# leok7v/sqz

Measured on AMD Instinct MI355X. Metric: encode MB/s + decode MB/s, 32KB window, batched blocks, 1/2/4/8 MI355X, higher is better.
Workload: dtype u8; 1 GPU; 4096 x 262144 B Zipf(s=1) byte blocks, window 2^15, one independent stream per block (BASELINE.json configs[2]); total_blocks=4096, blocks_per_gpu=4096, block_bytes=262144, win_bits=15, parallelism=1 rank; the N>1 runs shard this same batch (strong scaling), finder=index, device=AMD Radeon Graphics (gfx950:sramecc+:xnack-)

## Files before the change

sqz_amd/csrc/lz77_index.hip:

```cpp
#include "sqz_device.h"
#include "sqz_kernels.h"

namespace sqzk {

constexpr int kSharedGiveUp = 8;
constexpr int kXcds = 8;
constexpr int kSortThreads = 1024;
constexpr int kSortWaves = kSortThreads / kWave;

constexpr int kSortTile = 4 * kSortThreads;

constexpr int kSortBins = 1024;
constexpr int kSortCntRow = kSortBins + 2;
struct SortLds {
    uint32_t elem[kSortTile];
    uint16_t dig[kSortTile];
    uint16_t cnt[kSortWaves][kSortCntRow];
    uint32_t gbase[3][kSortBins];
    uint32_t delta[kSortBins];
    uint32_t wtot[kSortWaves];
};

struct __attribute__((packed)) U32u { uint32_t v; };

__device__ __forceinline__ uint32_t load_u32_unaligned(const uint8_t* p) {
    return reinterpret_cast<const U32u*>(p)->v;
}

__device__ __forceinline__ uint64_t peers_of(uint32_t digit, bool valid, int bits) {
    const uint64_t all = __ballot(valid);
    uint32_t lo = (uint32_t)all, hi = (uint32_t)(all >> 32);
#pragma unroll
    for (int bit = 0; bit < 10; bit++) {
        if (bit < bits) {
            const uint32_t mine = (uint32_t)((int32_t)(digit << (31 - bit)) >> 31);
            const uint64_t m = __ballot(mine != 0u);
            lo &= ~((uint32_t)m ^ mine);
            hi &= ~((uint32_t)(m >> 32) ^ mine);
        }
    }
    return ((uint64_t)hi << 32) | lo;
}

__device__ __forceinline__ uint32_t lanes_below(uint64_t mask) {
    return __builtin_amdgcn_mbcnt_hi((uint32_t)(mask >> 32),
                                     __builtin_amdgcn_mbcnt_lo((uint32_t)mask, 0u));
}

__device__ __forceinline__ uint32_t sort_key(const uint8_t* src, uint64_t bytes, uint32_t k) {
    return (uint64_t)k + 4 <= bytes ? (__builtin_bswap32(load_u32_unaligned(src + k)) >> 8)
                                    : (((uint32_t)src[k] << 16) | ((uint32_t)src[k + 1] << 8) | (uint32_t)src[k + 2]);
}

typedef uint32_t __attribute__((may_alias)) SortCntPair;

struct SortSec {
#ifdef SQZ_STATS
    uint64_t t[8] = {0, 0, 0, 0, 0, 0, 0, 0};
    uint64_t last = 0;
#endif
};
#ifdef SQZ_STATS
#define SORT_SEC(s, k) { const uint64_t n_ = __builtin_readcyclecounter(); (s).t[k] += n_ - (s).last; (s).last = n_; }
#define SORT_SEC_LOADS(s, k) { asm volatile("s_waitcnt vmcnt(0)" ::: "memory"); SORT_SEC(s, k) }
#else
#define SORT_SEC(s, k)
#define SORT_SEC_LOADS(s, k)
#endif

template <int kBits, bool kSmall>
__device__ __forceinline__ void sort_pass(SortLds& lds, const int pass, const uint8_t* __restrict__ src,
                                          const uint64_t bytes, const uint32_t count, const bool carry,
                                          const uint32_t* __restrict__ from, uint32_t* __restrict__ to, SortSec& sec) {
    constexpr int kDigits = 1 << kBits;
    constexpr int kTpd = kSortThreads / kDigits;
    constexpr int kWpt = kSortWaves / kTpd;
    const int tid = threadIdx.x;
    const int lane = tid & (kWave - 1);
    const int wave = __builtin_amdgcn_readfirstlane(tid >> 6);
    const bool first = kSmall ? kBits == 10 : pass == 0;
    uint32_t* const gbase = lds.gbase[pass];

    auto fetch = [&](uint32_t tile, uint32_t (&raw)[4]) {
#pragma unroll
        for (int j = 0; j < 4; j++) {
            const uint32_t k = tile + (uint32_t)(wave * 256 + j * kWave + lane);
            if (first) {
                const uint32_t last = (uint32_t)(bytes - 4);
                raw[j] = load_u32_unaligned(src + (k < last ? k : last));
            } else {
                raw[j] = from[k < count ? k : count - 1u];
            }
        }
    };
    auto key_from = [&](uint32_t raw, uint32_t k) {
        const uint32_t be = __builtin_bswap32(raw);
        return (uint64_t)k + 4 <= bytes ? be >> 8 : be & 0x00FFFFFFu;
    };
    auto decode = [&](uint32_t tile, const uint32_t (&raw)[4], uint32_t (&elem)[4], uint32_t (&digit)[4], bool (&valid)[4]) {
#pragma unroll
        for (int j = 0; j < 4; j++) {
            const uint32_t k = tile + (uint32_t)(wave * 256 + j * kWave + lane);
            valid[j] = k < count;
            const uint32_t pos = valid[j] ? (first ? k : raw[j]) : 0u;
            digit[j] = 0; elem[j] = pos;
            if (!valid[j]) { continue; }
            if (kSmall) {
                if (first) {
                    const uint32_t key = key_from(raw[j], k);
                    digit[j] = key & 0x3FFu;
                    elem[j] = pos | ((key >> 10) << 18);
                } else if (pass == 1) {
                    digit[j] = (pos >> 18) & 0x7Fu;
                } else {
                    digit[j] = pos >> 25;
                    elem[j] = pos & 0x3FFFFu;
                }
            } else if (first) {
                digit[j] = key_from(raw[j], k) & 0xFFu;
            } else if (pass == 1) {
                const uint32_t w = (uint32_t)src[pos] | ((uint32_t)src[pos + 1] << 8);
                digit[j] = w >> 8;
                if (carry) { elem[j] = pos | ((w & 0xFFu) << 24); }
            } else {
                digit[j] = carry ? (pos >> 24) : (uint32_t)src[pos];
                if (carry) { elem[j] = pos & 0x00FFFFFFu; }
            }
        }
    };

    uint32_t ahead[4], elem[4], digit[4], wrank[4];
    bool valid[4];
    fetch(0u, ahead);
    decode(0u, ahead, elem, digit, valid);
    SORT_SEC_LOADS(sec, 1)
    for (uint32_t tile = 0; tile < count; tile += (uint32_t)kSortTile) {
        const uint32_t n_tile = count - tile < (uint32_t)kSortTile ? count - tile : (uint32_t)kSortTile;
        fetch(tile + (uint32_t)kSortTile, ahead);
        {
            SortCntPair* const row = reinterpret_cast<SortCntPair*>(lds.cnt[wave]);
            for (int d = lane; d < kDigits / 2; d += kWave) { row[d] = 0u; }
        }
#pragma unroll
        for (int j = 0; j < 4; j++) {
            const uint64_t peers = peers_of(digit[j], valid[j], kBits);
            const uint32_t rank = lanes_below(peers);
            wrank[j] = valid[j] ? (uint32_t)lds.cnt[wave][digit[j]] + rank : 0u;
            __builtin_amdgcn_wave_barrier();
            if (valid[j] && rank == 0) {
                lds.cnt[wave][digit[j]] = (uint16_t)(lds.cnt[wave][digit[j]] + (uint32_t)__builtin_popcountll(peers));
            }
            __builtin_amdgcn_wave_barrier();
        }
        lds_barrier();
        SORT_SEC(sec, 2)
        const int sd = tid / kTpd;
        const int sw = (tid % kTpd) * kWpt;
        uint32_t c[kWpt], sum = 0;
#pragma unroll
        for (int i = 0; i < kWpt; i++) { c[i] = lds.cnt[sw + i][sd]; sum += c[i]; }
        const uint32_t incl = wave_scan(sum);
        if (lane == kWave - 1) { lds.wtot[wave] = incl; }
        lds_barrier();
        SORT_SEC(sec, 3)
        uint32_t at = wave_scan(lane < wave ? lds.wtot[lane] : 0u);
        at = (uint32_t)__builtin_amdgcn_readlane((int)at, kWave - 1) + incl - sum;
        const uint32_t run = at;
#pragma unroll
        for (int i = 0; i < kWpt; i++) { lds.cnt[sw + i][sd] = (uint16_t)at; at += c[i]; }
        const uint32_t run_end = kTpd > 1 ? (uint32_t)__shfl((int)at, lane | (kTpd - 1)) : at;
        if (tid % kTpd == 0) {
            const uint32_t g = gbase[sd];
            lds.delta[sd] = g - run;
            gbase[sd] = g + (run_end - run);
        }
        lds_barrier();
        SORT_SEC(sec, 4)
#pragma unroll
        for (int j = 0; j < 4; j++) {
            if (valid[j]) {
                const uint32_t slot = (uint32_t)lds.cnt[wave][digit[j]] + wrank[j];
                if (slot < (uint32_t)kSortTile) {
                    lds.elem[slot] = elem[j];
                    lds.dig[slot] = (uint16_t)digit[j];
                }
            }
        }
        lds_barrier();
        SORT_SEC(sec, 5)
#pragma unroll
        for (int j = 0; j < 4; j++) {
            const uint32_t slot = (uint32_t)(j * kSortThreads + tid);
            const uint32_t s = slot < n_tile ? slot : n_tile - 1u;
            const uint32_t dest = s + lds.delta[lds.dig[s]];
            to[dest < count ? dest : count - 1u] = lds.elem[s];
        }
        SORT_SEC(sec, 6)
        decode(tile + (uint32_t)kSortTile, ahead, elem, digit, valid);
        SORT_SEC_LOADS(sec, 1)
    }
    __threadfence_block();
    __syncthreads();
}

__global__ __launch_bounds__(kSortThreads)
void index_sort_kernel(const uint8_t* __restrict__ in,
                       const uint64_t* __restrict__ in_off,
                       uint32_t n_blocks,
                       uint32_t* __restrict__ buf_a,
                       uint32_t* __restrict__ buf_b,
                       uint64_t slots) {
    __shared__ SortLds lds;
    const uint32_t b = blockIdx.x;
    if (b >= n_blocks || in_off[b + 1] > slots) { return; }
    const int tid = threadIdx.x;
    const int lane = tid & (kWave - 1);
    const int wave = __builtin_amdgcn_readfirstlane(tid >> 6);

    const uint8_t* src = in + in_off[b];
    const uint64_t bytes = in_off[b + 1] - in_off[b];
    if (bytes < 3) { return; }
    const uint32_t count = (uint32_t)(bytes - 2);
    uint32_t* const pa = buf_a + in_off[b];
    uint32_t* const pb = buf_b + in_off[b];
    if (bytes == 3) {
        if (tid == 0) { pa[0] = 0u; }
        return;
    }
    const bool small = bytes <= (1u << 18);
    const bool carry = bytes <= (1u << 24);
    const int w0 = small ? 10 : 8, w1 = small ? 7 : 8, w2 = small ? 7 : 8;
    const int s1 = w0, s2 = w0 + w1;
    const uint32_t m0 = (1u << w0) - 1u, m1 = (1u << w1) - 1u;
    SortSec sec;
#ifdef SQZ_STATS
    sec.last = __builtin_readcyclecounter();
    const uint64_t sec_begin = sec.last;
#endif
    for (int d = tid; d < 3 * kSortBins; d += kSortThreads) { (&lds.gbase[0][0])[d] = 0; }
    __syncthreads();
    auto count_key = [&](uint32_t key) {
        atomicAdd(&lds.gbase[0][key & m0], 1u);
        atomicAdd(&lds.gbase[1][(key >> s1) & m1], 1u);
        atomicAdd(&lds.gbase[2][key >> s2], 1u);
    };
    const uint32_t quads = bytes >= 8 ? (uint32_t)((bytes - 8) / 4) + 1u : 0u;
    if ((uint32_t)tid < quads) {
        uint32_t lo = load_u32_unaligned(src + 4u * (uint32_t)tid), hi = load_u32_unaligned(src + 4u * (uint32_t)tid + 4u);
        for (uint32_t q = (uint32_t)tid; q < quads; q += (uint32_t)kSortThreads) {
            const uint64_t eight = ((uint64_t)hi << 32) | lo;
            const uint32_t nq = q + (uint32_t)kSortThreads < quads ? q + (uint32_t)kSortThreads : q;
            lo = load_u32_unaligned(src + 4u * nq); hi = load_u32_unaligned(src + 4u * nq + 4u);
#pragma unroll
            for (int j = 0; j < 4; j++) { count_key(__builtin_bswap32((uint32_t)(eight >> (8 * j))) >> 8); }
        }
    }
    for (uint32_t k = 4u * quads + (uint32_t)tid; k < count; k += (uint32_t)kSortThreads) { count_key(sort_key(src, bytes, k)); }
    __syncthreads();
    if (wave < 3) {
        uint32_t* const g = lds.gbase[wave];
        const int per = (1 << (wave == 0 ? w0 : wave == 1 ? w1 : w2)) / kWave;
        uint32_t sum = 0;
        for (int j = 0; j < per; j++) { sum += g[per * lane + j]; }
        uint32_t excl = wave_scan(sum) - sum;
        for (int j = 0; j < per; j++) { const uint32_t v = g[per * lane + j]; g[per * lane + j] = excl; excl += v; }
    }
    __syncthreads();
    SORT_SEC(sec, 0)

    if (small) {
        sort_pass<10, true>(lds, 0, src, bytes, count, carry, pb, pa, sec);
        for (int pass = 1; pass < 3; pass++) {
            sort_pass<7, true>(lds, pass, src, bytes, count, carry, pass == 1 ? pa : pb, pass == 1 ? pb : pa, sec);
        }
    } else {
        for (int pass = 0; pass < 3; pass++) {
            sort_pass<8, false>(lds, pass, src, bytes, count, carry, pass == 1 ? pa : pb, pass == 1 ? pb : pa, sec);
        }
    }
#ifdef SQZ_STATS
    if (tid == 0 && b == 1) {
        printf("sort block 1: cycles %llu: hist %llu; tiles: loads %llu rank %llu scan_a %llu scan_b %llu place %llu copy_out %llu\n",
               (unsigned long long)(sec.last - sec_begin), (unsigned long long)sec.t[0], (unsigned long long)sec.t[1],
               (unsigned long long)sec.t[2], (unsigned long long)sec.t[3], (unsigned long long)sec.t[4],
               (unsigned long long)sec.t[5], (unsigned long long)sec.t[6]);
    }
#endif
}

__global__ __launch_bounds__(256)
void index_match_kernel(const uint8_t* __restrict__ in,
                        const uint64_t* __restrict__ in_off,
                        uint32_t n_blocks, uint32_t window,
                        const uint32_t* __restrict__ sorted,
                        uint32_t* __restrict__ match, uint32_t groups, uint64_t slots) {
    const uint32_t xcd = blockIdx.x % (uint32_t)kXcds;
    const uint32_t local = blockIdx.x / (uint32_t)kXcds;
    const uint32_t b = (local / groups) * (uint32_t)kXcds + xcd;
    const uint32_t group = local % groups;
    if (b >= n_blocks || in_off[b + 1] > slots) { return; }
    const uint8_t* src = in + in_off[b];
    const uint64_t bytes = in_off[b + 1] - in_off[b];
    if (bytes < 3) { return; }
    const uint32_t n = (uint32_t)bytes;
    const uint32_t count = n - 2;
    const uint32_t* S = sorted + in_off[b];
    uint32_t* M = match + in_off[b];

    const int lane = (int)(threadIdx.x & (kWave - 1));
    const uint32_t pages = (count + (uint32_t)kWave - 1u) / (uint32_t)kWave;
    const uint32_t waves = groups * (blockDim.x / (uint32_t)kWave);
    const uint32_t per_wave = (pages + waves - 1u) / waves;
    const uint32_t wave_id = group * (blockDim.x / (uint32_t)kWave) + (threadIdx.x - (uint32_t)lane) / (uint32_t)kWave;
    const uint32_t page_lo = wave_id * per_wave;
    const uint32_t page_hi = page_lo + per_wave < pages ? page_lo + per_wave : pages;
    auto load16 = [&](uint32_t at, uint32_t& w0, uint32_t& w1, uint32_t& w2, uint32_t& w3) {
        if (at + 16 <= n) {
            w0 = load_u32_unaligned(src + at); w1 = load_u32_unaligned(src + at + 4);
            w2 = load_u32_unaligned(src + at + 8); w3 = load_u32_unaligned(src + at + 12);
        } else {
            uint32_t w[4] = {0, 0, 0, 0};
            for (uint32_t k = 0; k < 16 && at + k < n; k++) { w[k >> 2] |= (uint32_t)src[at + k] << (8 * (k & 3)); }
            w0 = w[0]; w1 = w[1]; w2 = w[2]; w3 = w[3];
        }
    };
    uint32_t prev_i = 0, prev0 = 0, prev1 = 0, prev2 = 0, prev3 = 0;
    if (page_lo > 0 && page_lo < page_hi) {
        prev_i = S[(page_lo - 1u) * (uint32_t)kWave + (uint32_t)lane];
        load16(prev_i, prev0, prev1, prev2, prev3);
    }
    for (uint32_t pg = page_lo; pg < page_hi; pg++) {
        const uint32_t r0 = pg * (uint32_t)kWave;
        const bool have_prev = pg > 0;
        const uint32_t r = r0 + (uint32_t)lane;
        const bool valid = r < count;
        const uint32_t i = valid ? S[r] : 0u;
        const uint32_t cap = (n - i) < (uint32_t)kLenMax ? (n - i) : (uint32_t)kLenMax;
        const uint32_t reach = i < window - 1 ? i : window - 1;
        uint32_t own0 = 0, own1 = 0, own2 = 0, own3 = 0;
        if (valid) { load16(i, own0, own1, own2, own3); }
        const uint32_t key = own0 & 0x00FFFFFFu;
        uint32_t best = 0, dist = 0;
        auto walk = [&](uint32_t q_from) {
            if (q_from == 0 || best >= cap) { return; }
            auto inside = [&](uint32_t r) {
                const uint32_t p = S[r];
                if (p + 4 > n) { return false; }
                return (load_u32_unaligned(src + p) & 0x00FFFFFFu) == key && i - p <= reach;
            };
            uint32_t q_lo;
            {
                uint32_t d = 4, bad = 0, good = q_from;
                bool open = true;
                while (open) {
                    if (d >= q_from) { bad = 0; open = false; if (inside(0)) { good = 0; } else { bad = 1; } }
                    else if (inside(q_from - d)) { good = q_from - d; d <<= 1; }
                    else { bad = q_from - d + 1; open = false; }
                }
                uint32_t lo = bad, hi = good;
                while (lo < hi) {
                    const uint32_t mid = lo + ((hi - lo) >> 1);
                    if (inside(mid)) { hi = mid; } else { lo = mid + 1; }
                }
                q_lo = lo;
            }
            uint8_t own_next = best >= (uint32_t)kLenMin ? src[i + best] : (uint8_t)0;
            for (uint32_t q = q_from; q > q_lo && best < cap; ) {
                q--;
                const uint32_t p = S[q];
                if (best >= (uint32_t)kLenMin && src[p + best] != own_next) { continue; }
                uint32_t k = 3;
                while (k < cap) {
                    if (i + k + 4 <= n) {
                        const uint32_t x = load_u32_unaligned(src + p + k) ^ load_u32_unaligned(src + i + k);
                        if (x != 0) { k += (uint32_t)__builtin_ctz(x) >> 3; break; }
                        k += 4;
                    } else {
                        if (src[p + k] != src[i + k]) { break; }
                        k++;
                    }
                }
                if (k > cap) { k = cap; }
                if (k > best) {
                    best = k; dist = i - p;
                    if (best < cap) { own_next = src[i + best]; }
                }
            }
        };
        const uint32_t key0 = (uint32_t)__builtin_amdgcn_readfirstlane((int)key);
        if (__ballot(valid && key == key0 && i + 16 <= n) == ~0ull) {
            bool done = false, deferred = false;
            uint32_t resume = 0;
            uint32_t page_base = r0, page = i, pb0 = own0, pb1 = own1, pb2 = own2, pb3 = own3;
            for (int64_t c = (int64_t)r0 + kWave - 2; c >= 0; c--) {
                if (c < (int64_t)page_base) {
                    page_base -= (uint32_t)kWave;
                    page = S[page_base + (uint32_t)lane];
                    load16(page, pb0, pb1, pb2, pb3);
                }
                const int at = (int)(c - (int64_t)page_base);
                const uint32_t pc = (uint32_t)__builtin_amdgcn_readlane((int)page, at);
                const bool below = (int64_t)r > c;
                const uint32_t d = i - pc;
                if (below && d > reach) { done = true; }
                if (__ballot(!done) == 0) { break; }
                const uint32_t c0 = (uint32_t)__builtin_amdgcn_readlane((int)pb0, at);
                if ((c0 & 0x00FFFFFFu) != key0) { break; }
                const uint32_t c1 = (uint32_t)__builtin_amdgcn_readlane((int)pb1, at);
                const uint32_t c2 = (uint32_t)__builtin_amdgcn_readlane((int)pb2, at);
                const uint32_t c3 = (uint32_t)__builtin_amdgcn_readlane((int)pb3, at);
                const uint32_t x0 = own0 ^ c0, x1 = own1 ^ c1, x2 = own2 ^ c2, x3 = own3 ^ c3;
                uint32_t len = x0 != 0 ? ((uint32_t)__builtin_ctz(x0) >> 3)
                             : x1 != 0 ? 4u + ((uint32_t)__builtin_ctz(x1) >> 3)
                             : x2 != 0 ? 8u + ((uint32_t)__builtin_ctz(x2) >> 3)
                             : x3 != 0 ? 12u + ((uint32_t)__builtin_ctz(x3) >> 3) : 16u;
                const bool want = below && !done;
                if (want && len == 16u && cap > 16u) {
                    deferred = true;
                    resume = (uint32_t)c + 1u;
                    done = true;
                } else {
                    if (len > cap) { len = cap; }
                    if (want && len > best) {
                        best = len; dist = d;
                        if (best >= cap) { done = true; }
                    }
                }
                if (__builtin_popcountll(__ballot(deferred)) >= kSharedGiveUp) {
                    if (!done) {
                        deferred = true;
                        resume = below ? (uint32_t)c : r;
                        done = true;
                    }
                    break;
                }
            }
            if (deferred) { walk(resume); }
            M[i] = best >= (uint32_t)kLenMin ? ((best << 16) | dist) : (key & 0xFFu);
            prev_i = i; prev0 = own0; prev1 = own1; prev2 = own2; prev3 = own3;
            continue;
        }
        bool done = !valid;
        bool later = false;
        uint32_t resume = 0;
        for (int k = 1; k <= kWave; k++) {
            const int from = lane - k;
            const bool in_cur = from >= 0;
            if (!done && !in_cur && !have_prev) { done = true; }
            if (__ballot(!done) == 0) { break; }
            const int addr = (from & (kWave - 1)) << 2;
            uint32_t pc = (uint32_t)__builtin_amdgcn_ds_bpermute(addr, (int)i);
            uint32_t c0 = (uint32_t)__builtin_amdgcn_ds_bpermute(addr, (int)own0);
            uint32_t c1 = (uint32_t)__builtin_amdgcn_ds_bpermute(addr, (int)own1);
            const bool back = __ballot(!done && !in_cur) != 0;
            if (back) {
                const uint32_t qc = (uint32_t)__builtin_amdgcn_ds_bpermute(addr, (int)prev_i);
                const uint32_t q0 = (uint32_t)__builtin_amdgcn_ds_bpermute(addr, (int)prev0);
                const uint32_t q1 = (uint32_t)__builtin_amdgcn_ds_bpermute(addr, (int)prev1);
                pc = in_cur ? pc : qc; c0 = in_cur ? c0 : q0; c1 = in_cur ? c1 : q1;
            }
            const uint32_t x0 = own0 ^ c0, x1 = own1 ^ c1;
            if (!done && (x0 & 0x00FFFFFFu) != 0) { done = true; }
            const uint32_t d = i - pc;
            if (!done && d > reach) { done = true; }
            uint32_t len = x0 != 0 ? ((uint32_t)__builtin_ctz(x0) >> 3) : x1 != 0 ? 4u + ((uint32_t)__builtin_ctz(x1) >> 3) : 8u;
            if (__ballot(!done && len == 8u && cap > 8u) != 0) {
                uint32_t c2 = (uint32_t)__builtin_amdgcn_ds_bpermute(addr, (int)own2);
                uint32_t c3 = (uint32_t)__builtin_amdgcn_ds_bpermute(addr, (int)own3);
                if (back) {
                    const uint32_t q2 = (uint32_t)__builtin_amdgcn_ds_bpermute(addr, (int)prev2);
                    const uint32_t q3 = (uint32_t)__builtin_amdgcn_ds_bpermute(addr, (int)prev3);
                    c2 = in_cur ? c2 : q2; c3 = in_cur ? c3 : q3;
                }
                const uint32_t x2 = own2 ^ c2, x3 = own3 ^ c3;
                if (len == 8u) {
                    len = x2 != 0 ? 8u + ((uint32_t)__builtin_ctz(x2) >> 3) : x3 != 0 ? 12u + ((uint32_t)__builtin_ctz(x3) >> 3) : 16u;
                }
            }
            if (!done) {
                if (len == 16u && cap > 16u) {
                    later = true;
                    resume = r - (uint32_t)k + 1u;
                    done = true;
                } else {
                    if (len > cap) { len = cap; }
                    if (len > best) {
                        best = len; dist = d;
                        if (best >= cap) { done = true; }
                    }
                    if (!done && k == kWave) {
                        later = true;
                        resume = r - (uint32_t)kWave;
                        done = true;
                    }
                }
            }
        }
        if (later) { walk(resume); }
        if (valid) { M[i] = best >= (uint32_t)kLenMin ? ((best << 16) | dist) : (key & 0xFFu); }
        prev_i = i; prev0 = own0; prev1 = own1; prev2 = own2; prev3 = own3;
    }
}

constexpr int kChunk = 32;
constexpr int kTile = kChunk * kWave;
constexpr int kChunkRow = kChunk + 1;

struct ParseLds {
    uint32_t m[kChunkRow * kWave];
};

__device__ __forceinline__ uint32_t parse_slot(uint32_t k) { return k + (k / (uint32_t)kChunk); }

__device__ __forceinline__ uint32_t parse_step(uint32_t w) {
    const uint32_t len = w >> 16;
    return len != 0 ? len : 1u;
}

__device__ __forceinline__ bool lazy_defers(uint32_t w, uint32_t w1) {
    const uint32_t len = w >> 16;
    return len >= (uint32_t)kLenMin && (w1 >> 16) > len;
}

constexpr int kTileRows = kTile / kWave;
__device__ __forceinline__ void parse_fetch(uint32_t (&w)[kTileRows], const uint32_t* __restrict__ M,
                                            const uint64_t tile, const uint64_t bytes, const int lane) {
    const uint64_t left = bytes - tile;
    const uint32_t last = left < (uint64_t)kTile ? (uint32_t)left - 1u : (uint32_t)kTile - 1u;
    const uint32_t* __restrict__ T = M + tile;
#pragma unroll
    for (int j = 0; j < kTileRows; j++) {
        const uint32_t k = (uint32_t)(j * kWave + lane);
        w[j] = T[k < last ? k : last];
    }
}

__device__ __forceinline__ uint32_t per_tile(uint32_t v) {
#ifndef SQZ_WAVE_EMU
    asm volatile("" : "+v"(v));
#endif
    return v;
}

struct ParseSec {
#ifdef SQZ_STATS
    uint64_t t[5] = {0, 0, 0, 0, 0};
    uint64_t last = 0;
#endif
};
#ifdef SQZ_STATS
#define PARSE_SEC(s, k) SORT_SEC(s, k)
#define PARSE_SEC_LOADS(s, k) SORT_SEC_LOADS(s, k)
#else
#define PARSE_SEC(s, k)
#define PARSE_SEC_LOADS(s, k)
#endif

template <bool kLazy>
__global__ __launch_bounds__(kWave)
void index_parse_kernel(const uint8_t* __restrict__ in,
                        const uint64_t* __restrict__ in_off,
                        uint32_t n_blocks,
                        const uint32_t* __restrict__ match,
                        uint32_t* __restrict__ tokens,
                        uint32_t* __restrict__ tok_count, uint64_t slots) {
    __shared__ ParseLds lds;
    const uint32_t b = blockIdx.x;
    if (b >= n_blocks) { return; }
    const int lane = threadIdx.x;
    if (in_off[b + 1] > slots) {
        if (lane == 0) { tok_count[b] = kRefused; }
        return;
    }
    const uint8_t* src = in + in_off[b];
    const uint64_t bytes = in_off[b + 1] - in_off[b];
    const uint32_t* M = match + in_off[b];
    uint32_t* tok = tokens + in_off[b];

    if (bytes == 0) {
        if (lane == 0) { tok_count[b] = 0; }
        return;
    }
    const uint32_t lit1 = (uint32_t)src[bytes - 1];
    const uint32_t lit2 = (uint32_t)src[bytes >= 2 ? bytes - 2 : 0];

    ParseSec sec;
#ifdef SQZ_STATS
    sec.last = __builtin_readcyclecounter();
    const uint64_t sec_begin = sec.last;
#endif
    uint32_t ntok = 0;
    uint32_t entry = 0;
    uint32_t fly[kTileRows];
    parse_fetch(fly, M, 0, bytes, lane);
    uint32_t fly_next = 0;
    auto fetch_next = [&](const uint64_t tile) __attribute__((always_inline)) {
        const uint64_t at = tile + (uint64_t)per_tile((uint32_t)kTile);
        fly_next = M[at < bytes ? at : bytes - 1];
    };
    if constexpr (kLazy) { fetch_next(0); }
    auto do_tile = [&](const uint64_t tile) __attribute__((always_inline)) -> bool {
        const uint64_t left = bytes - tile;
        const uint32_t have = left < (uint64_t)kTile ? (uint32_t)left : (uint32_t)kTile;
        if (entry >= have) { return false; }
        PARSE_SEC_LOADS(sec, 0)
        lds_barrier();
        const int t2 = left < (uint64_t)(kTile + 2) ? (int)left - 2 : kTile;
        uint32_t* const mine_at = &lds.m[parse_slot((uint32_t)lane)];
#pragma unroll
        for (int j = 0; j < kTileRows; j++) {
            const int tj = t2 - j * kWave;
            mine_at[j * (kWave + kWave / kChunk)] = lane < tj ? fly[j] : lane == tj ? lit2 : lit1;
        }
        uint32_t over = 0;
        if constexpr (kLazy) {
            over = left > (uint64_t)(kTile + 2) ? fly_next : 0u;
        }
        lds_barrier();
        const uint64_t ahead = tile + (uint64_t)kTile < bytes ? tile + (uint64_t)kTile : tile;
        parse_fetch(fly, M, ahead, bytes, lane);
        if constexpr (kLazy) { fetch_next(ahead); }
        PARSE_SEC(sec, 1)

        const uint32_t lo = (uint32_t)lane * (uint32_t)kChunk;
        const uint32_t room = have > lo ? (have - lo < (uint32_t)kChunk ? have - lo : (uint32_t)kChunk) : 0u;
        const uint32_t* row = &lds.m[lane * kChunkRow];
        uint32_t defer = 0;
        if constexpr (kLazy) {
            const uint32_t behind = lane + 1 < kWave ? lds.m[(lane + 1 < kWave ? lane + 1 : lane) * kChunkRow] : over;
            uint32_t w = row[0];
#pragma unroll 1
            for (int j0 = 0; j0 < kChunk; j0 += 8) {
#pragma unroll
                for (int j = 0; j < 8; j++) {
                    const uint32_t w1 = j0 + j + 1 < kChunk ? row[j0 + j + 1] : behind;
                    defer |= (lazy_defers(w, w1) ? 1u : 0u) << (j0 + j);
                    w = w1;
                }
            }
        }
        uint32_t guess = 0;
        uint32_t p = 0;
        while (p < room) {
            guess |= 1u << p;
            const uint32_t w = row[p];
            if constexpr (kLazy) { p += ((defer >> p) & 1u) != 0 ? 1u : parse_step(w); } else { p += parse_step(w); }
        }
        const uint32_t guess_out = lo + p;
        PARSE_SEC(sec, 2)

        uint32_t extra = 0;
        uint32_t from = (uint32_t)kChunk;
        uint32_t e = entry;
        while (e < have) {
            const uint32_t l = e / (uint32_t)kChunk;
            const uint32_t clo = l * (uint32_t)kChunk;
            const uint32_t g = (uint32_t)__builtin_amdgcn_readlane((int)guess, (int)l);
            uint32_t q = e - clo;
            if (((g >> q) & 1u) != 0) {
                e = (uint32_t)__builtin_amdgcn_readlane((int)guess_out, (int)l);
                if ((uint32_t)lane == l) { from = q; }
                continue;
            }
            const uint32_t croom = have - clo < (uint32_t)kChunk ? have - clo : (uint32_t)kChunk;
            uint32_t real = 0;
            do {
                real |= 1u << q;
                const uint32_t w = (uint32_t)__builtin_amdgcn_readfirstlane((int)lds.m[l * kChunkRow + q]);
                if constexpr (kLazy) {
                    const uint32_t dl = (uint32_t)__builtin_amdgcn_readlane((int)defer, (int)l);
                    q += ((dl >> q) & 1u) != 0 ? 1u : parse_step(w);
                } else {
                    q += parse_step(w);
                }
            } while (q < croom && ((g >> q) & 1u) == 0);
            const bool met = q < croom;
            e = met ? (uint32_t)__builtin_amdgcn_readlane((int)guess_out, (int)l) : clo + q;
            if ((uint32_t)lane == l) { extra = real; from = met ? q : (uint32_t)kChunk; }
        }
        const uint32_t mine = extra | (from < (uint32_t)kChunk ? guess & (~0u << from) : 0u);
        entry = e - (uint32_t)kTile;
        uint32_t give = 0, give_j0 = 0, give_j1 = 0, give_b0 = 0, give_b1 = 0;
        if constexpr (kLazy) {
            give = mine & defer;
            const uint32_t second = give & (give - 1u);
            give_j0 = give != 0 ? (uint32_t)__builtin_ctz(give) : 0u;
            give_j1 = second != 0 ? (uint32_t)__builtin_ctz(second) : give_j0;
            const uint64_t at0 = tile + (uint64_t)(lo + give_j0), at1 = tile + (uint64_t)(lo + give_j1);
            give_b0 = src[at0 < bytes ? at0 : bytes - 1];
            give_b1 = src[at1 < bytes ? at1 : bytes - 1];
        }
        PARSE_SEC(sec, 3)

        uint32_t mw[kChunk];
#pragma unroll
        for (int j = 0; j < kChunk; j++) { mw[j] = row[j]; }
        const uint32_t cnt = (uint32_t)__builtin_popcount(mine);
        const uint32_t incl = wave_scan(cnt);
        const uint32_t total = (uint32_t)__builtin_amdgcn_readlane((int)incl, kWave - 1);
        lds_barrier();
        uint32_t at = incl - cnt;
#pragma unroll
        for (int j = 0; j < kChunk; j++) {
            if ((mine >> j) & 1u) {
                lds.m[at++] = (mw[j] >> 16) != 0 ? (kTokMatch | mw[j]) : (mw[j] & 0xFFu);
            }
        }
        if constexpr (kLazy) {
            const uint32_t first = incl - cnt;
            auto slot_of = [&](uint32_t j) { return first + (uint32_t)__builtin_popcount(mine & ((1u << j) - 1u)); };
            uint32_t rest = give;
            if (rest != 0) { lds.m[slot_of(give_j0)] = give_b0; rest &= rest - 1u; }
            if (rest != 0) { lds.m[slot_of(give_j1)] = give_b1; rest &= rest - 1u; }
            while (rest != 0) {
                const uint32_t j = (uint32_t)__builtin_ctz(rest);
                rest &= rest - 1u;
                lds.m[slot_of(j)] = (uint32_t)src[tile + (uint64_t)(lo + j)];
            }
        }
        lds_barrier();
        uint32_t* const out = tok + ntok;
        const uint32_t last = total - 1u;
        const uint32_t ln = per_tile((uint32_t)lane);
#pragma unroll
        for (int j = 0; j < kTileRows; j++) {
            const uint32_t k = (uint32_t)(j * kWave) + ln;
            const uint32_t n = (k < last ? k : last) & (uint32_t)(kTile - 1);
            out[n] = lds.m[n];
        }
        ntok += total;
        PARSE_SEC(sec, 4)
        return true;
    };
    static_assert(kTile > kLenMax, "a token never reaches over a whole tile");
    if (do_tile(0)) {
        for (uint64_t tile = (uint64_t)kTile; tile < bytes; tile += (uint64_t)kTile) {
            if (!do_tile(tile)) { break; }
        }
    }
    if (lane == 0) { tok_count[b] = ntok; }
#ifdef SQZ_STATS
    if (lane == 0 && b == 1) {
        printf("parse block 1: cycles %llu: tiles: arrived %llu stage %llu guess %llu fixup %llu write %llu\n",
               (unsigned long long)(sec.last - sec_begin), (unsigned long long)sec.t[0], (unsigned long long)sec.t[1],
               (unsigned long long)sec.t[2], (unsigned long long)sec.t[3], (unsigned long long)sec.t[4]);
    }
#endif
}

#ifndef SQZ_DICT_THREADS
#define SQZ_DICT_THREADS 1024
#endif
constexpr int kDictThreads = SQZ_DICT_THREADS;
struct DictLds {
    uint8_t byte[kMaxWindow];
    uint16_t rank[kMaxWindow];
};

__global__ __launch_bounds__(kDictThreads)
void dict_match_kernel(const uint8_t* __restrict__ in,
                       const uint64_t* __restrict__ in_off,
                       uint32_t n_blocks, uint32_t window,
                       const uint8_t* __restrict__ dict, uint32_t D,
                       const uint32_t* __restrict__ dsorted,
                       uint32_t* __restrict__ match, uint64_t slots) {
    __shared__ __attribute__((aligned(16))) DictLds lds;
    const uint32_t tid = threadIdx.x;
    if (D == 0 || D >= (uint32_t)kMaxWindow) { return; }
    const uint32_t cnt = D >= 3 ? D - 2 : 0u;
    {
        const bool aligned = (reinterpret_cast<uintptr_t>(dict) & 15u) == 0;
        const uint32_t groups = aligned ? D / 16u : 0u;
        for (uint32_t g = tid; g < groups; g += (uint32_t)kDictThreads) {
            reinterpret_cast<uint4*>(lds.byte)[g] = reinterpret_cast<const uint4*>(dict)[g];
        }
        for (uint32_t k = groups * 16u + tid; k < (uint32_t)kMaxWindow; k += (uint32_t)kDictThreads) {
            lds.byte[k] = k < D ? dict[k] : (uint8_t)0;
        }
        const uint32_t quads = (cnt + 3u) / 4u;
        for (uint32_t g = tid; g < quads; g += (uint32_t)kDictThreads) {
            const uint4 v = reinterpret_cast<const uint4*>(dsorted)[g];
            SortCntPair* const two = reinterpret_cast<SortCntPair*>(lds.rank) + 2u * g;
            two[0] = (v.x & 0xFFFFu) | (v.y << 16);
            two[1] = (v.z & 0xFFFFu) | (v.w << 16);
        }
    }
    __syncthreads();
    auto lds_u32 = [&](uint32_t at) { return reinterpret_cast<const U32u*>(lds.byte + at)->v; };
    auto dkey = [&](uint32_t p) { return __builtin_bswap32(lds_u32(p)) >> 8; };
    const uint32_t reach = window - 1u;

    for (uint32_t b = blockIdx.x; b < n_blocks; b += gridDim.x) {
        if (in_off[b + 1] > slots) { continue; }
        const uint8_t* src = in + in_off[b];
        const uint64_t bytes = in_off[b + 1] - in_off[b];
        if (bytes < 3) { continue; }
        uint32_t* M = match + in_off[b];
        const uint64_t upto = bytes - 2 < (uint64_t)reach ? bytes - 2 : (uint64_t)reach;
        for (uint32_t i = tid; i < (uint32_t)upto; i += (uint32_t)kDictThreads) {
            const uint64_t left = bytes - i;
            const uint32_t cap = left < (uint64_t)kLenMax ? (uint32_t)left : (uint32_t)kLenMax;
            uint32_t best = M[i] >> 16;
            if (best >= cap) { continue; }
            const uint32_t q_min = D + i > reach ? D + i - reach : 0u;
            auto vbyte = [&](uint32_t v) { return v < D ? lds.byte[v] : src[v - D]; };
            auto extend = [&](uint32_t q) {
                const uint32_t in_d = D - q < cap ? D - q : cap;
                uint32_t k = 0;
                while (k < in_d) {
                    if (k + 4 <= in_d) {
                        const uint32_t x = lds_u32(q + k) ^ load_u32_unaligned(src + i + k);
                        if (x != 0) { return k + ((uint32_t)__builtin_ctz(x) >> 3); }
                        k += 4;
                    } else {
                        if (lds.byte[q + k] != src[i + k]) { return k; }
                        k++;
                    }
                }
                while (k < cap) {
                    const uint32_t s = q + k - D;
                    if (k + 4 <= cap) {
                        const uint32_t x = load_u32_unaligned(src + s) ^ load_u32_unaligned(src + i + k);
                        if (x != 0) { return k + ((uint32_t)__builtin_ctz(x) >> 3); }
                        k += 4;
                    } else {
                        if (src[s] != src[i + k]) { return k; }
                        k++;
                    }
                }
                return k;
            };
            uint32_t dist = 0;
            uint8_t own_next = best >= (uint32_t)kLenMin ? src[i + best] : (uint8_t)0;
            auto consider = [&](uint32_t q) {
                if (best >= (uint32_t)kLenMin && vbyte(q + best) != own_next) { return; }
                const uint32_t len = extend(q);
                if (len >= (uint32_t)kLenMin && len > best) {
                    best = len; dist = D + i - q;
                    if (best < cap) { own_next = src[i + best]; }
                }
            };
            if (D - 1u >= q_min) { consider(D - 1u); }
            if (D >= 2u && D - 2u >= q_min && best < cap) { consider(D - 2u); }
            if (cnt != 0 && best < cap) {
                const uint32_t key = sort_key(src, bytes, i);
                uint32_t lo = 0, hi = cnt;
                while (lo < hi) {
                    const uint32_t mid = lo + ((hi - lo) >> 1);
                    if (dkey(lds.rank[mid]) <= key) { lo = mid + 1; } else { hi = mid; }
                }
                uint32_t end = lo;
                lo = 0; hi = end;
                while (lo < hi) {
                    const uint32_t mid = lo + ((hi - lo) >> 1);
                    if (dkey(lds.rank[mid]) < key) { lo = mid + 1; } else { hi = mid; }
                }
                const uint32_t begin = lo;
                while (end > begin && best < cap) {
                    const uint32_t q = lds.rank[--end];
                    if (q < q_min) { break; }
                    consider(q);
                }
            }
            if (dist != 0) { M[i] = (best << 16) | dist; }
        }
    }
}

void launch_index_sort(const uint8_t* in, const uint64_t* in_off, uint32_t n_blocks,
                       uint32_t* buf_a, uint32_t* buf_b, uint64_t slots,
                       hipStream_t stream) {
    if (n_blocks == 0) { return; }
    hipLaunchKernelGGL(index_sort_kernel, dim3(n_blocks), dim3(kSortThreads), 0, stream,
                       in, in_off, n_blocks, buf_a, buf_b, slots);
}

void launch_index_match(const uint8_t* in, const uint64_t* in_off, uint32_t n_blocks,
                        uint32_t window, const uint32_t* sorted, uint32_t* match,
                        uint32_t match_groups, uint64_t slots, hipStream_t stream) {
    if (n_blocks == 0) { return; }
    if (match_groups < 1) { match_groups = 1; }
    const uint32_t rounded = (n_blocks + (uint32_t)kXcds - 1) / (uint32_t)kXcds * (uint32_t)kXcds;
    while ((uint64_t)match_groups * rounded > 0x7FFFFFFFull) { match_groups = (match_groups + 1) / 2; }
    hipLaunchKernelGGL(index_match_kernel, dim3(rounded * match_groups), dim3(256), 0, stream,
                       in, in_off, n_blocks, window, sorted, match, match_groups, slots);
}

void launch_index_parse(const uint8_t* in, const uint64_t* in_off, uint32_t n_blocks,
                        const uint32_t* match, uint32_t* tokens, uint32_t* tok_count,
                        uint64_t slots, hipStream_t stream) {
    if (n_blocks == 0) { return; }
    hipLaunchKernelGGL(index_parse_kernel<false>, dim3(n_blocks), dim3(kWave), 0, stream,
                       in, in_off, n_blocks, match, tokens, tok_count, slots);
}

void launch_index_parse_lazy(const uint8_t* in, const uint64_t* in_off, uint32_t n_blocks,
                             const uint32_t* match, uint32_t* tokens, uint32_t* tok_count,
                             uint64_t slots, hipStream_t stream) {
    if (n_blocks == 0) { return; }
    hipLaunchKernelGGL(index_parse_kernel<true>, dim3(n_blocks), dim3(kWave), 0, stream,
                       in, in_off, n_blocks, match, tokens, tok_count, slots);
}

void launch_dict_match(const uint8_t* in, const uint64_t* in_off, uint32_t n_blocks, uint32_t window,
                       const uint8_t* dict, uint32_t dict_bytes, const uint32_t* dict_sorted,
                       uint32_t* match, uint64_t slots, hipStream_t stream) {
    if (n_blocks == 0) { return; }
    const uint32_t grid = n_blocks < 1024u ? n_blocks : 1024u;
    hipLaunchKernelGGL(dict_match_kernel, dim3(grid), dim3(kDictThreads), 0, stream,
                       in, in_off, n_blocks, window, dict, dict_bytes, dict_sorted, match, slots);
}

}
```

Baseline: 15140 MB/s.

## Software-pipeline sorted-position and 16-byte loads in index match kernel

Restructures the match kernel's page loop so the sorted position and 16-byte window for the next page (and the position two pages ahead) are fetched before the current page is processed. The loads become single 128-bit loads clamped to the block tail, with a byte shift for lanes near the end, replacing the per-word and byte-loop loads. The candidate loops replace done/deferred branching with predicated boolean updates and 64-bit XOR/ctz comparisons, and invalid tail lanes now write a duplicate word instead of branching. The aim is to hide global-load latency and cut divergence, at the cost of more live registers and extra code for small blocks and the tail.

```diff
diff --git a/sqz_amd/csrc/lz77_index.hip b/sqz_amd/csrc/lz77_index.hip
--- a/sqz_amd/csrc/lz77_index.hip
+++ b/sqz_amd/csrc/lz77_index.hip
@@ -286,6 +286,30 @@
                (unsigned long long)sec.t[5], (unsigned long long)sec.t[6]);
     }
 #endif
+}
+
+struct __attribute__((packed)) U128u { uint32_t w[4]; };
+
+struct MatchSec {
+#ifdef SQZ_STATS
+    uint64_t t[4] = {0, 0, 0, 0};
+    uint64_t last = 0;
+#endif
+};
+#ifdef SQZ_STATS
+#define MATCH_SEC(s, k) SORT_SEC(s, k)
+#define MATCH_SEC_LOADS(s, k) SORT_SEC_LOADS(s, k)
+#else
+#define MATCH_SEC(s, k)
+#define MATCH_SEC_LOADS(s, k)
+#endif
+
+__device__ __forceinline__ void drop_bytes(uint32_t& w0, uint32_t& w1, uint32_t& w2, uint32_t& w3, uint32_t k) {
+    uint64_t lo = ((uint64_t)w1 << 32) | w0, hi = ((uint64_t)w3 << 32) | w2;
+    const uint32_t s = 8u * k;
+    if (s >= 64u) { lo = hi >> (s - 64u); hi = 0; }
+    else if (s != 0u) { lo = (lo >> s) | (hi << (64u - s)); hi >>= s; }
+    w0 = (uint32_t)lo; w1 = (uint32_t)(lo >> 32); w2 = (uint32_t)hi; w3 = (uint32_t)(hi >> 32);
 }
 
 __global__ __launch_bounds__(256)
@@ -314,192 +338,229 @@
     const uint32_t wave_id = group * (blockDim.x / (uint32_t)kWave) + (threadIdx.x - (uint32_t)lane) / (uint32_t)kWave;
     const uint32_t page_lo = wave_id * per_wave;
     const uint32_t page_hi = page_lo + per_wave < pages ? page_lo + per_wave : pages;
-    auto load16 = [&](uint32_t at, uint32_t& w0, uint32_t& w1, uint32_t& w2, uint32_t& w3) {
-        if (at + 16 <= n) {
-            w0 = load_u32_unaligned(src + at); w1 = load_u32_unaligned(src + at + 4);
-            w2 = load_u32_unaligned(src + at + 8); w3 = load_u32_unaligned(src + at + 12);
-        } else {
-            uint32_t w[4] = {0, 0, 0, 0};
-            for (uint32_t k = 0; k < 16 && at + k < n; k++) { w[k >> 2] |= (uint32_t)src[at + k] << (8 * (k & 3)); }
-            w0 = w[0]; w1 = w[1]; w2 = w[2]; w3 = w[3];
-        }
+    if (page_lo >= page_hi) { return; }
+    MatchSec sec;
+#ifdef SQZ_STATS
+    sec.last = __builtin_readcyclecounter();
+    const uint64_t sec_begin = sec.last;
+#endif
+    auto walk = [&](const uint32_t q_from, const uint32_t i, const uint32_t key, const uint32_t cap, const uint32_t reach,
+                    uint32_t& best, uint32_t& dist) __attribute__((always_inline)) {
+        if (q_from == 0 || best >= cap) { return; }
+        auto inside = [&](uint32_t r) {
+            const uint32_t p = S[r];
+            if (p + 4 > n) { return false; }
+            return (load_u32_unaligned(src + p) & 0x00FFFFFFu) == key && i - p <= reach;
+        };
+        uint32_t q_lo;
+        {
+            uint32_t d = 4, bad = 0, good = q_from;
+            bool open = true;
+            while (open) {
+                if (d >= q_from) { bad = 0; open = false; if (inside(0)) { good = 0; } else { bad = 1; } }
+                else if (inside(q_from - d)) { good = q_from - d; d <<= 1; }
+                else { bad = q_from - d + 1; open = false; }
+            }
+            uint32_t lo = bad, hi = good;
+            while (lo < hi) {
+                const uint32_t mid = lo + ((hi - lo) >> 1);
+                if (inside(mid)) { hi = mid; } else { lo = mid + 1; }
+            }
+            q_lo = lo;
+        }
+        uint8_t own_next = best >= (uint32_t)kLenMin ? src[i + best] : (uint8_t)0;
+        for (uint32_t q = q_from; q > q_lo && best < cap; ) {
+            q--;
+            const uint32_t p = S[q];
+            if (best >= (uint32_t)kLenMin && src[p + best] != own_next) { continue; }
+            uint32_t k = 3;
+            while (k < cap) {
+                if (i + k + 4 <= n) {
+                    const uint32_t x = load_u32_unaligned(src + p + k) ^ load_u32_unaligned(src + i + k);
+                    if (x != 0) { k += (uint32_t)__builtin_ctz(x) >> 3; break; }
+                    k += 4;
+                } else {
+                    if (src[p + k] != src[i + k]) { break; }
+                    k++;
+                }
+            }
+            if (k > cap) { k = cap; }
+            if (k > best) {
+                best = k; dist = i - p;
+                if (best < cap) { own_next = src[i + best]; }
+            }
+        }
+    };
+    if (n < 16u) {
+        if ((uint32_t)lane < count) {
+            const uint32_t i = S[lane];
+            const uint32_t key = (uint32_t)src[i] | ((uint32_t)src[i + 1] << 8) | ((uint32_t)src[i + 2] << 16);
+            const uint32_t cap = n - i;
+            const uint32_t reach = i < window - 1 ? i : window - 1;
+            uint32_t best = 0, dist = 0;
+            walk((uint32_t)lane, i, key, cap, reach, best, dist);
+            M[i] = best >= (uint32_t)kLenMin ? ((best << 16) | dist) : (key & 0xFFu);
+        }
+        return;
+    }
+    const uint32_t tail = n - 16u;
+    const uint32_t page_last = page_hi - 1u;
+    auto fetch_pos = [&](uint32_t pg) {
+        const uint32_t r = (pg < page_last ? pg : page_last) * (uint32_t)kWave + (uint32_t)lane;
+        return S[r < count - 1u ? r : count - 1u];
+    };
+    auto fetch16 = [&](uint32_t at) { return *reinterpret_cast<const U128u*>(src + (at < tail ? at : tail)); };
+    auto settle16 = [&](uint32_t at, const U128u& got, uint32_t& w0, uint32_t& w1, uint32_t& w2, uint32_t& w3) {
+        w0 = got.w[0]; w1 = got.w[1]; w2 = got.w[2]; w3 = got.w[3];
+        if (__ballot(at > tail) != 0) { drop_bytes(w0, w1, w2, w3, at > tail ? at - tail : 0u); }
     };
     uint32_t prev_i = 0, prev0 = 0, prev1 = 0, prev2 = 0, prev3 = 0;
-    if (page_lo > 0 && page_lo < page_hi) {
-        prev_i = S[(page_lo - 1u) * (uint32_t)kWave + (uint32_t)lane];
-        load16(prev_i, prev0, prev1, prev2, prev3);
-    }
-    for (uint32_t pg = page_lo; pg < page_hi; pg++) {
+
+    auto do_page = [&](const uint32_t pg, const uint32_t i, const uint32_t own0, const uint32_t own1,
+                       const uint32_t own2, const uint32_t own3) __attribute__((always_inline)) {
+        MATCH_SEC_LOADS(sec, 0)
         const uint32_t r0 = pg * (uint32_t)kWave;
         const bool have_prev = pg > 0;
         const uint32_t r = r0 + (uint32_t)lane;
         const bool valid = r < count;
-        const uint32_t i = valid ? S[r] : 0u;
         const uint32_t cap = (n - i) < (uint32_t)kLenMax ? (n - i) : (uint32_t)kLenMax;
         const uint32_t reach = i < window - 1 ? i : window - 1;
-        uint32_t own0 = 0, own1 = 0, own2 = 0, own3 = 0;
-        if (valid) { load16(i, own0, own1, own2, own3); }
         const uint32_t key = own0 & 0x00FFFFFFu;
         uint32_t best = 0, dist = 0;
-        auto walk = [&](uint32_t q_from) {
-            if (q_from == 0 || best >= cap) { return; }
-            auto inside = [&](uint32_t r) {
-                const uint32_t p = S[r];
-                if (p + 4 > n) { return false; }
-                return (load_u32_unaligned(src + p) & 0x00FFFFFFu) == key && i - p <= reach;
-            };
-            uint32_t q_lo;
-            {
-                uint32_t d = 4, bad = 0, good = q_from;
-                bool open = true;
-                while (open) {
-                    if (d >= q_from) { bad = 0; open = false; if (inside(0)) { good = 0; } else { bad = 1; } }
-                    else if (inside(q_from - d)) { good = q_from - d; d <<= 1; }
-                    else { bad = q_from - d + 1; open = false; }
-                }
-                uint32_t lo = bad, hi = good;
-                while (lo < hi) {
-                    const uint32_t mid = lo + ((hi - lo) >> 1);
-                    if (inside(mid)) { hi = mid; } else { lo = mid + 1; }
-                }
-                q_lo = lo;
-            }
-            uint8_t own_next = best >= (uint32_t)kLenMin ? src[i + best] : (uint8_t)0;
-            for (uint32_t q = q_from; q > q_lo && best < cap; ) {
-                q--;
-                const uint32_t p = S[q];
-                if (best >= (uint32_t)kLenMin && src[p + best] != own_next) { continue; }
-                uint32_t k = 3;
-                while (k < cap) {
-                    if (i + k + 4 <= n) {
-                        const uint32_t x = load_u32_unaligned(src + p + k) ^ load_u32_unaligned(src + i + k);
-                        if (x != 0) { k += (uint32_t)__builtin_ctz(x) >> 3; break; }
-                        k += 4;
-                    } else {
-                        if (src[p + k] != src[i + k]) { break; }
-                        k++;
-                    }
-                }
-                if (k > cap) { k = cap; }
-                if (k > best) {
-                    best = k; dist = i - p;
-                    if (best < cap) { own_next = src[i + best]; }
-                }
-            }
-        };
+        bool later = false;
+        uint32_t resume = 0;
         const uint32_t key0 = (uint32_t)__builtin_amdgcn_readfirstlane((int)key);
-        if (__ballot(valid && key == key0 && i + 16 <= n) == ~0ull) {
-            bool done = false, deferred = false;
-            uint32_t resume = 0;
+        if (__ballot(valid && key == key0 && i <= tail) == ~0ull) {
+            bool alive = true;
             uint32_t page_base = r0, page = i, pb0 = own0, pb1 = own1, pb2 = own2, pb3 = own3;
+            const uint64_t own_lo = ((uint64_t)own1 << 32) | own0, own_hi = ((uint64_t)own3 << 32) | own2;
             for (int64_t c = (int64_t)r0 + kWave - 2; c >= 0; c--) {
                 if (c < (int64_t)page_base) {
                     page_base -= (uint32_t)kWave;
                     page = S[page_base + (uint32_t)lane];
-                    load16(page, pb0, pb1, pb2, pb3);
+                    settle16(page, fetch16(page), pb0, pb1, pb2, pb3);
                 }
                 const int at = (int)(c - (int64_t)page_base);
                 const uint32_t pc = (uint32_t)__builtin_amdgcn_readlane((int)page, at);
                 const bool below = (int64_t)r > c;
                 const uint32_t d = i - pc;
-                if (below && d > reach) { done = true; }
-                if (__ballot(!done) == 0) { break; }
+                alive &= !(below & (d > reach));
+                if (__ballot(alive) == 0) { break; }
                 const uint32_t c0 = (uint32_t)__builtin_amdgcn_readlane((int)pb0, at);
                 if ((c0 & 0x00FFFFFFu) != key0) { break; }
                 const uint32_t c1 = (uint32_t)__builtin_amdgcn_readlane((int)pb1, at);
                 const uint32_t c2 = (uint32_t)__builtin_amdgcn_readlane((int)pb2, at);
                 const uint32_t c3 = (uint32_t)__builtin_amdgcn_readlane((int)pb3, at);
-                const uint32_t x0 = own0 ^ c0, x1 = own1 ^ c1, x2 = own2 ^ c2, x3 = own3 ^ c3;
-                uint32_t len = x0 != 0 ? ((uint32_t)__builtin_ctz(x0) >> 3)
-                             : x1 != 0 ? 4u + ((uint32_t)__builtin_ctz(x1) >> 3)
-                             : x2 != 0 ? 8u + ((uint32_t)__builtin_ctz(x2) >> 3)
-                             : x3 != 0 ? 12u + ((uint32_t)__builtin_ctz(x3) >> 3) : 16u;
-                const bool want = below && !done;
-                if (want && len == 16u && cap > 16u) {
-                    deferred = true;
-                    resume = (uint32_t)c + 1u;
-                    done = true;
-                } else {
-                    if (len > cap) { len = cap; }
-                    if (want && len > best) {
-                        best = len; dist = d;
-                        if (best >= cap) { done = true; }
-                    }
-                }
-                if (__builtin_popcountll(__ballot(deferred)) >= kSharedGiveUp) {
-                    if (!done) {
-                        deferred = true;
+                const uint64_t x_lo = own_lo ^ (((uint64_t)c1 << 32) | c0), x_hi = own_hi ^ (((uint64_t)c3 << 32) | c2);
+                uint32_t len = x_lo != 0 ? ((uint32_t)__builtin_ctzll(x_lo) >> 3)
+                             : x_hi != 0 ? 8u + ((uint32_t)__builtin_ctzll(x_hi) >> 3) : 16u;
+                const bool want = below & alive;
+                const bool full = want & (len == 16u) & (cap > 16u);
+                later |= full;
+                resume = full ? (uint32_t)c + 1u : resume;
+                alive &= !full;
+                len = len > cap ? cap : len;
+                const bool better = want & !full & (len > best);
+                best = better ? len : best;
+                dist = better ? d : dist;
+                alive &= best < cap;
+                if (__builtin_popcountll(__ballot(later)) >= kSharedGiveUp) {
+                    if (alive) {
+                        later = true;
                         resume = below ? (uint32_t)c : r;
-                        done = true;
                     }
                     break;
                 }
             }
-            if (deferred) { walk(resume); }
-            M[i] = best >= (uint32_t)kLenMin ? ((best << 16) | dist) : (key & 0xFFu);
-            prev_i = i; prev0 = own0; prev1 = own1; prev2 = own2; prev3 = own3;
-            continue;
-        }
-        bool done = !valid;
-        bool later = false;
-        uint32_t resume = 0;
-        for (int k = 1; k <= kWave; k++) {
-            const int from = lane - k;
-            const bool in_cur = from >= 0;
-            if (!done && !in_cur && !have_prev) { done = true; }
-            if (__ballot(!done) == 0) { break; }
-            const int addr = (from & (kWave - 1)) << 2;
-            uint32_t pc = (uint32_t)__builtin_amdgcn_ds_bpermute(addr, (int)i);
-            uint32_t c0 = (uint32_t)__builtin_amdgcn_ds_bpermute(addr, (int)own0);
-            uint32_t c1 = (uint32_t)__builtin_amdgcn_ds_bpermute(addr, (int)own1);
-            const bool back = __ballot(!done && !in_cur) != 0;
-            if (back) {
-                const uint32_t qc = (uint32_t)__builtin_amdgcn_ds_bpermute(addr, (int)prev_i);
-                const uint32_t q0 = (uint32_t)__builtin_amdgcn_ds_bpermute(addr, (int)prev0);
-                const uint32_t q1 = (uint32_t)__builtin_amdgcn_ds_bpermute(addr, (int)prev1);
-                pc = in_cur ? pc : qc; c0 = in_cur ? c0 : q0; c1 = in_cur ? c1 : q1;
-            }
-            const uint32_t x0 = own0 ^ c0, x1 = own1 ^ c1;
-            if (!done && (x0 & 0x00FFFFFFu) != 0) { done = true; }
-            const uint32_t d = i - pc;
-            if (!done && d > reach) { done = true; }
-            uint32_t len = x0 != 0 ? ((uint32_t)__builtin_ctz(x0) >> 3) : x1 != 0 ? 4u + ((uint32_t)__builtin_ctz(x1) >> 3) : 8u;
-            if (__ballot(!done && len == 8u && cap > 8u) != 0) {
-                uint32_t c2 = (uint32_t)__builtin_amdgcn_ds_bpermute(addr, (int)own2);
-                uint32_t c3 = (uint32_t)__builtin_amdgcn_ds_bpermute(addr, (int)own3);
+        } else {
+            bool alive = valid;
+            const uint64_t own_lo = ((uint64_t)own1 << 32) | own0;
+            for (int k = 1; k <= kWave; k++) {
+                const int from = lane - k;
+                const bool in_cur = from >= 0;
+                alive &= in_cur | have_prev;
+                if (__ballot(alive) == 0) { break; }
+                const int addr = (from & (kWave - 1)) << 2;
+                uint32_t pc = (uint32_t)__builtin_amdgcn_ds_bpermute(addr, (int)i);
+                uint32_t c0 = (uint32_t)__builtin_amdgcn_ds_bpermute(addr, (int)own0);
+                uint32_t c1 = (uint32_t)__builtin_amdgcn_ds_bpermute(addr, (int)own1);
+                const bool back = __ballot(alive & !in_cur) != 0;
                 if (back) {
-                    const uint32_t q2 = (uint32_t)__builtin_amdgcn_ds_bpermute(addr, (int)prev2);
-                    const uint32_t q3 = (uint32_t)__builtin_amdgcn_ds_bpermute(addr, (int)prev3);
-                    c2 = in_cur ? c2 : q2; c3 = in_cur ? c3 : q3;
-                }
-                const uint32_t x2 = own2 ^ c2, x3 = own3 ^ c3;
-                if (len == 8u) {
-                    len = x2 != 0 ? 8u + ((uint32_t)__builtin_ctz(x2) >> 3) : x3 != 0 ? 12u + ((uint32_t)__builtin_ctz(x3) >> 3) : 16u;
-                }
-            }
-            if (!done) {
-                if (len == 16u && cap > 16u) {
-                    later = true;
-                    resume = r - (uint32_t)k + 1u;
-                    done = true;
-                } else {
-                    if (len > cap) { len = cap; }
-                    if (len > best) {
-                        best = len; dist = d;
-                        if (best >= cap) { done = true; }
+                    const uint32_t qc = (uint32_t)__builtin_amdgcn_ds_bpermute(addr, (int)prev_i);
+                    const uint32_t q0 = (uint32_t)__builtin_amdgcn_ds_bpermute(addr, (int)prev0);
+                    const uint32_t q1 = (uint32_t)__builtin_amdgcn_ds_bpermute(addr, (int)prev1);
+                    pc = in_cur ? pc : qc; c0 = in_cur ? c0 : q0; c1 = in_cur ? c1 : q1;
+                }
+                const uint64_t x = own_lo ^ (((uint64_t)c1 << 32) | c0);
+                const uint32_t d = i - pc;
+                alive &= (((uint32_t)x & 0x00FFFFFFu) == 0u) & (d <= reach);
+                uint32_t len = x != 0 ? ((uint32_t)__builtin_ctzll(x) >> 3) : 8u;
+                if (__ballot(alive & (len == 8u) & (cap > 8u)) != 0) {
+                    uint32_t c2 = (uint32_t)__builtin_amdgcn_ds_bpermute(addr, (int)own2);
+                    uint32_t c3 = (uint32_t)__builtin_amdgcn_ds_bpermute(addr, (int)own3);
+                    if (back) {
+                        const uint32_t q2 = (uint32_t)__builtin_amdgcn_ds_bpermute(addr, (int)prev2);
+                        const uint32_t q3 = (uint32_t)__builtin_amdgcn_ds_bpermute(addr, (int)prev3);
+                        c2 = in_cur ? c2 : q2; c3 = in_cur ? c3 : q3;
                     }
-                    if (!done && k == kWave) {
-                        later = true;
-                        resume = r - (uint32_t)kWave;
-                        done = true;
-                    }
-                }
-            }
-        }
-        if (later) { walk(resume); }
-        if (valid) { M[i] = best >= (uint32_t)kLenMin ? ((best << 16) | dist) : (key & 0xFFu); }
+                    const uint64_t x_hi = (((uint64_t)own3 << 32) | own2) ^ (((uint64_t)c3 << 32) | c2);
+                    const uint32_t more = x_hi != 0 ? 8u + ((uint32_t)__builtin_ctzll(x_hi) >> 3) : 16u;
+                    len = len == 8u ? more : len;
+                }
+                const bool full = alive & (len == 16u) & (cap > 16u);
+                later |= full;
+                resume = full ? r - (uint32_t)k + 1u : resume;
+                alive &= !full;
+                len = len > cap ? cap : len;
+                const bool better = alive & (len > best);
+                best = better ? len : best;
+                dist = better ? d : dist;
+                alive &= best < cap;
+            }
+            resume = alive ? r - (uint32_t)kWave : resume;
+            later |= alive;
+        }
+        MATCH_SEC(sec, 1)
+        if (later) { walk(resume, i, key, cap, reach, best, dist); }
+        MATCH_SEC(sec, 2)
+        const uint32_t word = best >= (uint32_t)kLenMin ? ((best << 16) | dist) : (key & 0xFFu);
+        const uint32_t ranks = count - r0;
+        const uint32_t last_word = (uint32_t)__builtin_amdgcn_readlane((int)word, (int)(ranks < (uint32_t)kWave ? ranks - 1u : (uint32_t)kWave - 1u));
+        M[i] = valid ? word : last_word;
+        MATCH_SEC(sec, 3)
         prev_i = i; prev0 = own0; prev1 = own1; prev2 = own2; prev3 = own3;
-    }
+    };
+
+    uint32_t pos_cur = fetch_pos(page_lo);
+    uint32_t pos_nxt = fetch_pos(page_lo + 1u);
+    if (page_lo > 0) {
+        prev_i = S[(page_lo - 1u) * (uint32_t)kWave + (uint32_t)lane];
+        settle16(prev_i, fetch16(prev_i), prev0, prev1, prev2, prev3);
+    }
+    U128u got_cur = fetch16(pos_cur);
+    {
+        const uint32_t pos_far = fetch_pos(page_lo + 2u);
+        const U128u got_nxt = fetch16(pos_nxt);
+        uint32_t own0, own1, own2, own3;
+        settle16(pos_cur, got_cur, own0, own1, own2, own3);
+        do_page(page_lo, pos_cur, own0, own1, own2, own3);
+        pos_cur = pos_nxt; pos_nxt = pos_far; got_cur = got_nxt;
+    }
+    for (uint32_t pg = page_lo + 1u; pg < page_hi; pg++) {
+        const uint32_t pos_far = fetch_pos(pg + 2u);
+        const U128u got_nxt = fetch16(pos_nxt);
+        uint32_t own0, own1, own2, own3;
+        settle16(pos_cur, got_cur, own0, own1, own2, own3);
+        do_page(pg, pos_cur, own0, own1, own2, own3);
+        pos_cur = pos_nxt; pos_nxt = pos_far; got_cur = got_nxt;
+    }
+#ifdef SQZ_STATS
+    if (threadIdx.x == 0 && b == 1 && group == 0) {
+        printf("match block 1: cycles %llu: loads %llu candidates %llu own_walks %llu store %llu\n",
+               (unsigned long long)(sec.last - sec_begin), (unsigned long long)sec.t[0], (unsigned long long)sec.t[1],
+               (unsigned long long)sec.t[2], (unsigned long long)sec.t[3]);
+    }
+#endif
 }
 
 constexpr int kChunk = 32;
```

After: 15340 MB/s, median of 6. 1.01x the previous value.
